# patrickltobing/shallow-wavenet

Hardware: AMD Instinct MI355X
Metric: decoded samples/sec (22.05 kHz Laplacian AR decode, whole job) (higher is better)
Workload: dtype f32

## Files before the change

shallow_wavenet_amd/csrc/swn_decode_bl6w.hip:

```cpp
#include <type_traits>
#include "swn_decode_bl6_common.hpp"
#include "swn_decode_internal.hpp"

#ifndef SWN_RES_SLICE
#define SWN_RES_SLICE 0
#endif
#ifndef SWN_ROTATE
#define SWN_ROTATE 1
#endif

namespace {

using namespace swn_bl6;

constexpr int NG = 256;
constexpr int S = 128;
constexpr int O1 = 128;

template <int LPC_, bool EXT_>
struct Tw {
    static constexpr int LPC = LPC_;
    static constexpr bool EXT = EXT_;
    using Ext = Tw<LPC_, true>;
    static constexpr int NO = 2 + LPC_;
    static constexpr int WN = cmax(1, LPC_) + 1;
    static constexpr int ring_len(int l) { return pow2ceil((1 << l) + 1); }
    static constexpr int ring_off(int l) { int o = 0; for (int i = 0; i < l; ++i) o += ring_len(i) * H; return o; }
    static constexpr int PF = L * 2 * H;
    static constexpr int NZC = 64, NZB = 4;
    static constexpr int o_ring = 0;
    static constexpr int o_hcat = o_ring + ring_off(L);
    static constexpr int o_gp = o_hcat + L * H;
    static constexpr int o_bx = o_gp + 2 * PF;
    static constexpr int o_bd = o_bx + L * 2 * H;
    static constexpr int o_old = o_bd + L * 2 * H;
    static constexpr int o_wup = o_old + 2 * L * 2 * H;
    static constexpr int o_skip = o_wup + 256;
    static constexpr int o_p2 = o_skip + S;
    static constexpr int o_tnz = o_p2 + 4 * NO;
    static constexpr int o_cz = o_tnz + r4(NZB * NZC);
    static constexpr int o_w2 = o_cz + 5 * H;
    static constexpr int o_bias = o_w2 + NO * S + r4(NO);
    static constexpr int o_w1 = o_bias + S + O1;
    static constexpr int o_wl = o_w1 + 8 * O1 * 16;
    static constexpr int o_h0w = o_wl + 8 * NG * 4;
    static constexpr int o_end = o_h0w + 3 * H;
    static constexpr size_t lds_bytes = (size_t)o_end * sizeof(float);
    static constexpr int sess_old = ring_off(L);
    static constexpr int sess_win = sess_old + 2 * L * 2 * H;
    static constexpr int sess_floats = sess_win + r4(WN);
};

__device__ __forceinline__ float sum_quads(float v) {
    v += dpp_f<0x124>(v);
    v += dpp_f<0x128>(v);
    float w = v;
    asm("s_nop 1\n\tv_permlane16_swap_b32 %0, %1" : "+v"(v), "+v"(w));
    v += w;
    w = v;
    asm("s_nop 1\n\tv_permlane32_swap_b32 %0, %1" : "+v"(v), "+v"(w));
    return v + w;
}
__device__ __forceinline__ float quad_sum_by_parity(float own, float other) {
    float s = own + dpp_f<0xB1>(other);
    s += dpp_f<0x4E>(s);
    return s;
}
struct NoWork { __device__ __forceinline__ void operator()() const {} };
template <class T, int LAYER, int NQ = 2, class BEHIND = NoWork>
__device__ __forceinline__ void layer_a(float* lds, const float (&w)[2][16], const int q, const float wj, const int pb, const int po,
                                        const int ta, const float* xr, BEHIND&& behind = NoWork{}) {
    constexpr bool ROT = !std::is_same<typename std::decay<BEHIND>::type, NoWork>::value;
    const int o = ta >> 2, p = ta & 3, pr = p & 1;
    const float e_old = lds[T::o_old + po + LAYER * 2 * H + pr * H + o];
    const float g_gp = lds[T::o_gp + pb + LAYER * 2 * H + pr * H + o], g_bx = lds[T::o_bx + LAYER * 2 * H + pr * H + o];
    const float e_hp = xr[o];
    static_assert(NQ >= 0 && NQ <= 4, "early quads");
    float4 xq[4];
    if constexpr (ROT) {
#pragma unroll
        for (int m = 0; m < NQ; ++m) xq[m] = *reinterpret_cast<const float4*>(xr + 16 * p + 4 * m);
        __builtin_amdgcn_sched_barrier(0);
        behind();
        __builtin_amdgcn_sched_barrier(0);
    }
    const float e_gx = fmaf(wj, g_gp, g_bx);
    float az = 0.f, ac = 0.f;
#pragma unroll
    for (int m = 0; m < 4; ++m) {
        float4 x;
        if (ROT && m < NQ) x = xq[m];
        else x = *reinterpret_cast<const float4*>(xr + 16 * p + 4 * m);
        az = fmaf(w[0][4 * m], x.x, az); ac = fmaf(w[1][4 * m], x.x, ac);
        az = fmaf(w[0][4 * m + 1], x.y, az); ac = fmaf(w[1][4 * m + 1], x.y, ac);
        az = fmaf(w[0][4 * m + 2], x.z, az); ac = fmaf(w[1][4 * m + 2], x.z, ac);
        az = fmaf(w[0][4 * m + 3], x.w, az); ac = fmaf(w[1][4 * m + 3], x.w, ac);
    }
    const float sq = quad_sum_by_parity(pr ? ac : az, pr ? az : ac);
    __builtin_amdgcn_sched_barrier(0);
    if (p < 2) {
        const float sa = sq + e_old;
        const float v = e_gx * sa;
        const float e = exp_c(p == 0 ? -v : -2.f * fminf(fabsf(v), 64.f));
        const float r = rcp_c(1.f + e);
        const float res = p == 0 ? r : copysignf((1.f - e) * r, v);
        const float c = dpp_f<0xF5>(res);
        if (p == 0) {
            const float hn = (1.f - res) * c + res * e_hp;
            if (LAYER + 1 < L) {
                constexpr int R2 = T::ring_len(LAYER + 1 < L ? LAYER + 1 : LAYER);
                lds[T::o_ring + T::ring_off(LAYER + 1 < L ? LAYER + 1 : LAYER) + (q & (R2 - 1)) * H + o] = hn;
            }
            lds[T::o_hcat + LAYER * H + o] = hn;
        }
    }
    __builtin_amdgcn_sched_barrier(0);
}

template <class T, int LAYER, int MB = 4>
__device__ __forceinline__ void older_sum(const float* lds, const float (&w)[2][16], const int qn, const int tb, float& az, float& ac) {
    constexpr int dil = 1 << LAYER;
    constexpr int R = T::ring_len(LAYER);
    const int p = tb & 3;
    const float* ring = lds + T::o_ring + T::ring_off(LAYER);
    az = 0.f; ac = 0.f;
#pragma unroll
    for (int m = 0; m < 4; ++m) {
        const float4 x = *reinterpret_cast<const float4*>(ring + ((qn - dil) & (R - 1)) * H + 16 * p + 4 * m);
        float4 w0, w1;
        if (LAYER < L - 1) {
            w0 = make_float4(w[0][4 * m], w[0][4 * m + 1], w[0][4 * m + 2], w[0][4 * m + 3]);
            w1 = make_float4(w[1][4 * m], w[1][4 * m + 1], w[1][4 * m + 2], w[1][4 * m + 3]);
        } else {
            w0 = *reinterpret_cast<const float4*>(lds + T::o_wl + (m * NG + tb) * 4);
            w1 = *reinterpret_cast<const float4*>(lds + T::o_wl + ((4 + m) * NG + tb) * 4);
        }
        az = fmaf(w0.x, x.x, az); ac = fmaf(w1.x, x.x, ac);
        az = fmaf(w0.y, x.y, az); ac = fmaf(w1.y, x.y, ac);
        az = fmaf(w0.z, x.z, az); ac = fmaf(w1.z, x.z, ac);
        az = fmaf(w0.w, x.w, az); ac = fmaf(w1.w, x.w, ac);
        if (MB < 4 && m % MB == MB - 1) __builtin_amdgcn_sched_barrier(0);
    }
    az = sum4(az); ac = sum4(ac);
}
template <class T, int LAYER>
__device__ __forceinline__ void older_store(float* lds, const int qn, const int tb, const float az, const float ac) {
    const int o = tb >> 2, p = tb & 3, pr = p & 1;
    lds[T::o_old + (qn & 1) * (L * 2 * H) + LAYER * 2 * H + pr * H + o] = (p == 0 ? az : ac) + lds[T::o_bd + LAYER * 2 * H + pr * H + o];
}
template <class T, int LAYER, int MB = 4>
__device__ __forceinline__ void older_b(float* lds, const float (&w)[2][16], const int qn, const int tb) {
    float az, ac;
    older_sum<T, LAYER, MB>(lds, w, qn, tb, az, ac);
    if ((tb & 3) < 2) older_store<T, LAYER>(lds, qn, tb, az, ac);
}
template <class T>
__device__ __forceinline__ void older_last_rows(const float* lds, const int qn, const int tb, float4 (&x)[2], float4 (&w)[2][2]) {
    constexpr int LAYER = L - 1, dil = 1 << LAYER, R = T::ring_len(LAYER);
    const float* row = lds + T::o_ring + T::ring_off(LAYER) + ((qn - dil) & (R - 1)) * H + 16 * (tb & 3);
#pragma unroll
    for (int m = 0; m < 2; ++m) {
        x[m] = *reinterpret_cast<const float4*>(row + 4 * m);
        w[m][0] = *reinterpret_cast<const float4*>(lds + T::o_wl + (m * NG + tb) * 4);
        w[m][1] = *reinterpret_cast<const float4*>(lds + T::o_wl + ((4 + m) * NG + tb) * 4);
    }
}
template <class T>
__device__ __forceinline__ void older_last_x(float* lds, const float4 (&xe)[2], const float4 (&we)[2][2], const int qn, const int tb) {
    constexpr int LAYER = L - 1, dil = 1 << LAYER, R = T::ring_len(LAYER);
    const float* row = lds + T::o_ring + T::ring_off(LAYER) + ((qn - dil) & (R - 1)) * H + 16 * (tb & 3);
    float az = 0.f, ac = 0.f;
#pragma unroll
    for (int m = 0; m < 4; ++m) {
        float4 x, w0, w1;
        if (m < 2) { x = xe[m]; w0 = we[m][0]; w1 = we[m][1]; }
        else {
            x = *reinterpret_cast<const float4*>(row + 4 * m);
            w0 = *reinterpret_cast<const float4*>(lds + T::o_wl + (m * NG + tb) * 4);
            w1 = *reinterpret_cast<const float4*>(lds + T::o_wl + ((4 + m) * NG + tb) * 4);
        }
        az = fmaf(w0.x, x.x, az); ac = fmaf(w1.x, x.x, ac);
        az = fmaf(w0.y, x.y, az); ac = fmaf(w1.y, x.y, ac);
        az = fmaf(w0.z, x.z, az); ac = fmaf(w1.z, x.z, ac);
        az = fmaf(w0.w, x.w, az); ac = fmaf(w1.w, x.w, ac);
        if (m == 1) __builtin_amdgcn_sched_barrier(0);
    }
    az = sum4(az); ac = sum4(ac);
    if ((tb & 3) < 2) older_store<T, LAYER>(lds, qn, tb, az, ac);
}
template <int... LS> struct Layers {};
template <class T, int NW, int... LS>
__device__ __forceinline__ void older_bn(Layers<LS...>, float* lds, const float (&w)[NW][2][16], const int qn, const int tb) {
    static_assert(((LS < NW) && ...), "register-resident halves only");
    float az[sizeof...(LS)], ac[sizeof...(LS)];
    int k = 0;
    ((older_sum<T, LS>(lds, w[LS], qn, tb, az[k], ac[k]), ++k), ...);
    if ((tb & 3) < 2) {
        k = 0;
        ((older_store<T, LS>(lds, qn, tb, az[k], ac[k]), ++k), ...);
    }
}

template <class T, int LAYER>
__device__ __forceinline__ void older_rows(const float* lds, const int qn, const int tb, float4 (&x)[4]) {
    constexpr int dil = 1 << LAYER;
    constexpr int R = T::ring_len(LAYER);
    const float* row = lds + T::o_ring + T::ring_off(LAYER) + ((qn - dil) & (R - 1)) * H + 16 * (tb & 3);
#pragma unroll
    for (int m = 0; m < 4; ++m) x[m] = *reinterpret_cast<const float4*>(row + 4 * m);
}
__device__ __forceinline__ void older_sum_x(const float (&w)[2][16], const float4 (&x)[4], float& az, float& ac) {
    az = 0.f; ac = 0.f;
#pragma unroll
    for (int m = 0; m < 4; ++m) {
        az = fmaf(w[0][4 * m], x[m].x, az); ac = fmaf(w[1][4 * m], x[m].x, ac);
        az = fmaf(w[0][4 * m + 1], x[m].y, az); ac = fmaf(w[1][4 * m + 1], x[m].y, ac);
        az = fmaf(w[0][4 * m + 2], x[m].z, az); ac = fmaf(w[1][4 * m + 2], x[m].z, ac);
        az = fmaf(w[0][4 * m + 3], x[m].w, az); ac = fmaf(w[1][4 * m + 3], x[m].w, ac);
    }
    az = sum4(az); ac = sum4(ac);
}
template <class T, int... LS>
__device__ __forceinline__ void older_rows_n(Layers<LS...>, const float* lds, const int qn, const int tb, float4 (&x)[sizeof...(LS)][4]) {
    int k = 0;
    ((older_rows<T, LS>(lds, qn, tb, x[k]), ++k), ...);
}
template <class T, int NW, int... LS>
__device__ __forceinline__ void older_bn_x(Layers<LS...>, float* lds, const float (&w)[NW][2][16], const float4 (&x)[sizeof...(LS)][4],
                                           const int qn, const int tb) {
    static_assert(((LS < NW) && ...), "register-resident halves only");
    float az[sizeof...(LS)], ac[sizeof...(LS)];
    int k = 0;
    ((older_sum_x(w[LS], x[k], az[k], ac[k]), ++k), ...);
    if ((tb & 3) < 2) {
        k = 0;
        ((older_store<T, LS>(lds, qn, tb, az[k], ac[k]), ++k), ...);
    }
}

template <int LAYER>
__device__ __forceinline__ void skip_issue_b(__amdgpu_buffer_rsrc_t wsk2, float4 (&wsl)[8], const int tb, const unsigned step0) {
    const int r = tb >> 2, hp = tb & 3;
#pragma unroll
    for (int ps = 0; ps < 2; ++ps)
#pragma unroll
        for (int mm = 0; mm < 4; ++mm)
            wsl[ps * 4 + mm] = buf_ld4(wsk2, (unsigned)((r + 64 * ps) * 4 + hp) * 16u, (unsigned)((LAYER * 4 + mm) * S) * 64u + step0);
}
template <class T, int LAYER, bool REQ = true>
__device__ __forceinline__ void skip_roll_b(const float* lds, __amdgpu_buffer_rsrc_t wsk2, const float4 (&wcur)[8], float4 (&wnext)[8],
                                            float (&sacc)[2], const int tb, const unsigned step0) {
    static_assert(LAYER >= 1 && LAYER < L, "slice LAYER - 1 in flight, slice LAYER to request");
    const int r = tb >> 2, hp = tb & 3;
    float4 xs[4];
#pragma unroll
    for (int mm = 0; mm < 4; ++mm) xs[mm] = *reinterpret_cast<const float4*>(lds + T::o_hcat + (LAYER - 1) * H + 16 * mm + 4 * hp);
#pragma unroll
    for (int mm = 0; mm < 4; ++mm) {
#pragma unroll
        for (int ps = 0; ps < 2; ++ps) {
            const float4 x = xs[mm], w = wcur[ps * 4 + mm];
            sacc[ps] = fmaf(w.x, x.x, sacc[ps]); sacc[ps] = fmaf(w.y, x.y, sacc[ps]);
            sacc[ps] = fmaf(w.z, x.z, sacc[ps]); sacc[ps] = fmaf(w.w, x.w, sacc[ps]);
        }
        __builtin_amdgcn_sched_barrier(0);
#pragma unroll
        for (int ps = 0; ps < 2; ++ps)
            if (REQ) wnext[ps * 4 + mm] = buf_ld4(wsk2, (unsigned)((r + 64 * ps) * 4 + hp) * 16u, (unsigned)((LAYER * 4 + mm) * S) * 64u + step0);
        __builtin_amdgcn_sched_barrier(0);
    }
    asm volatile("" : "+v"(sacc[0]), "+v"(sacc[1]));
}
template <class T>
__device__ __forceinline__ void skip_last_b(float* lds, const float4 (&wsl)[8], const float (&sacc)[2], const int tb) {
    const int r = tb >> 2, hp = tb & 3;
    float part[2][4];
#pragma unroll
    for (int mm = 0; mm < 4; ++mm) {
        const float4 x = *reinterpret_cast<const float4*>(lds + T::o_hcat + (L - 1) * H + 16 * mm + 4 * hp);
#pragma unroll
        for (int ps = 0; ps < 2; ++ps) {
            const float4 w = wsl[ps * 4 + mm];
            part[ps][mm] = fmaf(w.w, x.w, fmaf(w.z, x.z, fmaf(w.y, x.y, w.x * x.x)));
        }
    }
    float s[2];
#pragma unroll
    for (int ps = 0; ps < 2; ++ps) s[ps] = sacc[ps] + ((part[ps][0] + part[ps][1]) + (part[ps][2] + part[ps][3]));
    const float t0 = s[0] + dpp_f<0xB1>(s[0]), t1 = s[1] + dpp_f<0xB1>(s[1]);
    const float v = (hp < 2 ? t0 : t1) + dpp_f<0x4E>(hp < 2 ? t1 : t0);
    if ((hp & 1) == 0) lds[T::o_skip + r + 32 * hp] = fmaxf(v, 0.f);
}

using OlderMerged = Layers<3, 4>;
using OlderOut1 = Layers<0, 1, 2>;

template <class T, bool GA, bool STREAM, bool POOL = false>
__device__ __forceinline__ void decode_body(const Bl6Args& a, float* lds) {
    constexpr bool EXT = T::EXT;
    static_assert(!STREAM || EXT, "streamed chunks run the extended mode");
    constexpr bool grpA = GA;
    const int tid = threadIdx.x, b = POOL ? 0 : blockIdx.x;
    __builtin_assume(GA ? tid < NG : tid >= NG);
    const int tg = tid & (NG - 1);
    const float* __restrict__ P = a.P;
    const int U = a.U;
    const int s0 = STREAM ? a.step0 : 0;
    const bool resume = STREAM && a.resume;
    const int fb0 = STREAM ? s0 / U : 0;

    for (int e = tid; e < T::o_end; e += NT) lds[e] = 0.f;
    __syncthreads();
    for (int e = tid; e < L * 2 * H; e += NT) {
        lds[T::o_bx + e] = P[a.y.bx + e];
        const float bd = P[a.y.bd + e];
        lds[T::o_bd + e] = bd;
        lds[T::o_old + e] = bd;
    }
    for (int e = tid; e < U; e += NT) lds[T::o_wup + e] = P[a.y.wup + e];
    for (int e = tid; e < H; e += NT) lds[T::o_cz + e] = P[a.y.cb + e];
    for (int e = tid; e < S; e += NT) lds[T::o_bias + e] = P[a.y.bsk + e];
    for (int e = tid; e < O1; e += NT) lds[T::o_bias + S + e] = P[a.y.b1 + e];
    for (int e = tid; e < 2 * H; e += NT) { lds[T::o_cz + H + e] = P[a.y.cv + e]; lds[T::o_cz + 3 * H + e] = P[a.y.cc + e]; }
    for (int e = tid; e < T::NO * S; e += NT) lds[T::o_w2 + e] = P[a.y.w2 + (size_t)(e / S) * r4(S) + (e % S)];
    for (int e = tid; e < T::NO; e += NT) lds[T::o_w2 + T::NO * S + e] = P[a.y.b2 + e];
    for (int e = tid; e < 8 * O1 * 16; e += NT) lds[T::o_w1 + e] = P[a.y.w12 + e];
    const __amdgpu_buffer_rsrc_t condr =
        make_rsrc(a.cond + (size_t)b * a.Tf * a.N, (unsigned)((size_t)a.Tf * a.N * sizeof(float)));
    auto load_frame = [&](int fr) {
        float* dst = lds + T::o_gp + (fr & 1) * T::PF;
#pragma unroll
        for (int it = 0; it < (T::PF / 4 + NT - 1) / NT; ++it) {
            const int e4 = it * NT + tid;
            if (e4 < T::PF / 4)
                *reinterpret_cast<float4*>(dst + 4 * e4) =
                    buf_ld4(condr, (unsigned)tid * 16u, (unsigned)(fr * a.N * 4 + it * NT * 16));
        }
    };
    for (int fr = fb0; fr < fb0 + 2 && fr < a.Tf; ++fr) load_frame(fr);
    constexpr int NWR = grpA ? L : L - 1;
    float wreg[NWR][2][16];
    {
        const int o = tg >> 2, p = tg & 3, k = grpA ? 1 : 0;
#pragma unroll
        for (int l = 0; l < L; ++l)
#pragma unroll
            for (int r = 0; r < 2; ++r) {
                const float4* src = reinterpret_cast<const float4*>(P + a.y.wd + (((size_t)l * 2 * H + o + r * H) * 2 + k) * H + 16 * p);
#pragma unroll
                for (int v = 0; v < 4; ++v) {
                    const float4 t = src[v];
                    if (l == L - 1 && !grpA) {
                        *reinterpret_cast<float4*>(lds + T::o_wl + ((r * 4 + v) * NG + tg) * 4) = t;
                    } else {
                        float (&wr)[16] = wreg[l < NWR ? l : 0][r];
                        wr[4 * v] = t.x; wr[4 * v + 1] = t.y; wr[4 * v + 2] = t.z; wr[4 * v + 3] = t.w;
                    }
                }
            }
    }
    __syncthreads();
    const float* sess_b = STREAM ? a.sess + (size_t)b * T::sess_floats : nullptr;
    int tcp = tid;
    asm volatile("" : "+v"(tcp));
    if (resume) {
        for (int e = tcp; e < T::ring_off(L); e += NT) lds[T::o_ring + e] = sess_b[e];
        for (int e = tcp; e < 2 * L * 2 * H; e += NT) lds[T::o_old + e] = sess_b[T::sess_old + e];
        __syncthreads();
    }

    int fb = fb0, tb0 = fb0 * U;
    const int n_pro = RF;
    auto cond_taps = [&](int q, float& wj, int& pb) {
        const int t0 = q - RF;
        const int tlo = t0 < 0 ? 0 : t0;
        if (tlo >= tb0 + U) {
            fb += 1; tb0 += U;
            if (fb + 1 < a.Tf) load_frame(fb + 1);
        }
        int rel = tlo - tb0;
        int fsel = fb;
        if (rel >= U) { rel -= U; fsel = fb + 1; }
        rel = rel < U ? rel : U - 1;
        wj = lds[T::o_wup + rel];
        pb = (fsel & 1) * T::PF;
    };

    auto input_seed = [&](int q) {
        if (tid < H) {
            const int o = tid;
            float acc = c_b;
#pragma unroll
            for (int k = 0; k < 2; ++k) {
                const int r = q - (1 - k);
                if (r >= 0) acc += fmaf(k ? c_v1 : c_v0, 0.f, k ? c_c1 : c_c0);
            }
            lds[T::o_ring + (q & 1) * H + o] = ssign(acc);
        }
    };
    float win[T::WN];
#pragma unroll
    for (int k = 0; k < T::WN; ++k) win[k] = 0.f;
    if (EXT && a.seed) win[T::WN - 1] = reinterpret_cast<const float*>(a.seed)[b];
    if (resume) {
#pragma unroll
        for (int k = 0; k < T::WN; ++k) win[k] = sess_b[T::sess_win + k];
    }
    const int wv = __builtin_amdgcn_readfirstlane(tg >> 6);
    float kcb = 0.f, kv0 = 0.f, kv1 = 0.f, kc0 = 0.f, kc1 = 0.f;
    if (grpA) { const int o = tg & (H - 1); kcb = c_b; kv0 = c_v0; kv1 = c_v1; kc0 = c_c0; kc1 = c_c1; }
    auto h0_row = [&](int qn) -> int {
        return wv == 0 ? T::o_ring + (qn & 1) * H : T::o_h0w + (wv - 1) * H;
    };
    auto input_gen = [&](int row) {
        if constexpr (grpA) {
            float acc = kcb;
            acc += fmaf(kv0, win[T::WN - 2], kc0);
            acc += fmaf(kv1, win[T::WN - 1], kc1);
            lds[row + (tg & (H - 1))] = ssign(acc);
            lds_fence_compiler();
        }
    };
    float e_next = 0.f;
    auto noise_load = [&](int c) {
        const int step = c * T::NZC + tid - 64;
        if (step < a.n_steps) e_next = a.noise[(size_t)b * a.n_steps + step];
    };
    auto noise_chunk = [&](int c) {
        if (grpA && tid >= 64 && tid < 128) {
            const int k = tid - 64, step = c * T::NZC + k;
            if (step < a.n_steps) {
                const float e = EXT ? swn_noise_laplace_at(a.nz, b, step, s0 + step, 0, a.n_steps, 1) : e_next;
                const float sg = (e > 0.f) ? 1.f : ((e < 0.f) ? -1.f : 0.f);
                lds[T::o_tnz + (c & (T::NZB - 1)) * T::NZC + k] = sg * log1pf(-2.f * fabsf(e));
            }
            if (!EXT) noise_load(c + 1);
        }
    };
    if (!EXT && grpA && tid >= 64 && tid < 128) noise_load(0);
    noise_chunk(0);
    noise_chunk(1);

    const __amdgpu_buffer_rsrc_t wsk2 = make_rsrc(P + a.y.wsk2, (unsigned)(L * S * 64 * sizeof(float)));
    constexpr bool NEWFORM = !EXT && T::LPC == 0;
    constexpr int RES = (grpA || !NEWFORM) ? -1 : SWN_RES_SLICE;
    static_assert(RES == -1 || RES == 0 || RES == L - 1, "the first or the last slice");
    float4 wres[8];
    if constexpr (RES == 0) skip_issue_b<0>(wsk2, wres, tg, 0u);
    if constexpr (RES == L - 1) skip_issue_b<L - 1>(wsk2, wres, tg, 0u);

#ifdef SWN_STAMP
    unsigned long long tw[9] = {0, 0, 0, 0, 0, 0, 0, 0, 0}, tv[6] = {0, 0, 0, 0, 0, 0}, tstep = 0, tlast = 0, tbeg = 0;
#define SWN_BAR(k) { tw[k] += __builtin_amdgcn_s_memtime() - tlast; lds_barrier(); tlast = __builtin_amdgcn_s_memtime(); }
#define SWN_WAIT_STAMP(k) { asm volatile("" :: "v"(wsl[0].x)); tv[k] += __builtin_amdgcn_s_memtime() - tlast; }
#define SWN_PRE(k) { tw[k] += __builtin_amdgcn_s_memtime() - tlast; asm volatile("s_waitcnt lgkmcnt(0)" ::: "memory"); }
#define SWN_BAR_KEEP(k, N) { lds_barrier_keep<N>(); tlast = __builtin_amdgcn_s_memtime(); }
#else
#define SWN_BAR(k) lds_barrier();
#define SWN_WAIT_STAMP(k)
#define SWN_PRE(k)
#define SWN_BAR_KEEP(k, N) lds_barrier_keep<N>();
#endif
#define SWN_PHASE_WORK(LAYER, GEN, X0)                                                                                \
    if constexpr (grpA) layer_a<T, LAYER>(lds, wreg[LAYER], q, wj, pb, po, tg,                                         \
                                          LAYER == 0 ? (X0) : lds + T::o_ring + T::ring_off(LAYER) +                   \
                                                                  (q & (T::ring_len(LAYER) - 1)) * H);                 \
    else {                                                                                                             \
        if (GEN) {    \
                      \
                      \
                      \
            if (LAYER == 0) { if (RES != 0) skip_issue_b<0>(wsk2, wsl, tg, step0); }                                   \
            else if (LAYER == 1 && RES == 0) skip_roll_b<T, 1>(lds, wsk2, wres, wsl, sacc, tg, step0);                 \
            else { SWN_WAIT_STAMP(LAYER > 0 ? LAYER - 1 : 0)                                                           \
                   skip_roll_b<T, (LAYER > 0 ? LAYER : 1), !(LAYER == L - 1 && RES == L - 1)>(lds, wsk2, wsl, wsl, sacc, tg, step0); } \
            __builtin_amdgcn_sched_barrier(0);                                                                         \
        }                                                                                                              \
        if (!(GEN)) older_b<T, LAYER>(lds, wreg[LAYER < NWR ? LAYER : 0], q + 1, tg);                                  \
        else if (LAYER == 0) older_bn<T>(OlderMerged{}, lds, wreg, q + 1, tg);                                         \
        __builtin_amdgcn_sched_barrier(0);                                                                             \
    }
#define SWN_PHASE(LAYER, GEN, X0) SWN_PHASE_WORK(LAYER, GEN, X0) if (GEN) { SWN_BAR(LAYER) } else lds_barrier();

#pragma unroll 1
    for (int q = resume ? n_pro : 0; q < n_pro; ++q) {
        float wj; int pb;
        float4 wsl[8]; float sacc[2]; const unsigned step0 = 0;
        cond_taps(q, wj, pb);
        const int po = (q & 1) * (L * 2 * H);
        input_seed(q);
        lds_barrier();
        const float* x0 = lds + T::o_ring + (q & 1) * H;
        SWN_PHASE(0, false, x0) SWN_PHASE(1, false, x0) SWN_PHASE(2, false, x0) SWN_PHASE(3, false, x0)
        SWN_PHASE(4, false, x0) SWN_PHASE(5, false, x0)
        (void)wsl; (void)sacc; (void)step0;
    }

    int rel_c = s0 - fb0 * U;
    bool fill_c = false;
    float wj_c = 0.f;
    int pb_c = 0, po_c = 0, x0_c = 0;
    auto taps_ahead = [&](int qn) {
        wj_c = lds[T::o_wup + rel_c];
        pb_c = (fb & 1) * T::PF;
        po_c = (qn & 1) * (L * 2 * H);
        x0_c = h0_row(qn);
        asm volatile("" : "+s"(pb_c), "+s"(po_c), "+s"(x0_c));
    };
    auto frame_advance = [&]() {
        rel_c += 1;
        const bool cross = rel_c >= U;
        if (cross) { rel_c = 0; fb += 1; }
        fill_c = cross && fb + 1 < a.Tf;
    };
    if constexpr (grpA) taps_ahead(RF + s0);
    input_gen(x0_c);
#ifdef SWN_STAMP
    tlast = tbeg = __builtin_amdgcn_s_memtime();
#endif
    constexpr bool ROT = SWN_ROTATE && NEWFORM;
    constexpr int ROTQ = 2;
    float sv_p = 0.f, acc_p = 0.f;
    const __amdgpu_buffer_rsrc_t outr =
        make_rsrc(reinterpret_cast<float*>(a.out) + (size_t)b * a.n_steps, (unsigned)((size_t)a.n_steps * sizeof(float)));
    const __amdgpu_buffer_rsrc_t headr =
        make_rsrc(HEADS_ON && a.heads ? a.heads + (size_t)b * a.n_steps * T::NO : nullptr,
                  HEADS_ON && a.heads ? (unsigned)((size_t)a.n_steps * T::NO * sizeof(float)) : 0u);
    auto store_step = [&](const int ip) __attribute__((always_inline)) {
        if constexpr (grpA && ROT) {
            if (tid == 0) __builtin_amdgcn_raw_buffer_store_b32(__builtin_bit_cast(unsigned, sv_p), outr, 0u, (unsigned)ip * 4u, 0);
            if (wv == 0 && (tg & 63) < T::NO)
                __builtin_amdgcn_raw_buffer_store_b32(__builtin_bit_cast(unsigned, acc_p), headr, (unsigned)(tg & 63) * 4u,
                                                      (unsigned)(ip * T::NO) * 4u, 0);
        } else if constexpr (grpA) {
            if (tid == 0) reinterpret_cast<float*>(a.out)[(size_t)b * a.n_steps + (size_t)ip] = sv_p;
            if (HEADS_ON && a.heads && wv == 0 && (tg & 63) < T::NO) a.heads[((size_t)b * a.n_steps + ip) * T::NO + (tg & 63)] = acc_p;
        }
    };
    auto gen_step = [&](const int i) __attribute__((always_inline)) {
        const int q = RF + s0 + i;
        const float wj = wj_c;
        const int pb = pb_c, po = po_c;
        if constexpr (grpA && !ROT) {
            if (fill_c) load_frame(fb + 1);
        }
        auto behind0 = [&]() __attribute__((always_inline)) {
            if ((i & (T::NZC - 1)) == 0) noise_chunk((i >> 6) + 2);
            if (fill_c) load_frame(fb + 1);
            if (i > 0) store_step(i - 1);
        };
        float4 wsl[8];
        float sacc[2] = {0.f, 0.f};
        if constexpr (!grpA) {
            const float bs0 = lds[T::o_bias + (tg >> 2)], bs1 = lds[T::o_bias + (tg >> 2) + 64];
            if ((tg & 3) == 0) { sacc[0] = bs0; sacc[1] = bs1; }
        }
        unsigned step0 = 0;
        asm volatile("" : "+s"(step0));
        const float* x0 = lds + x0_c;
        if constexpr (grpA && ROT) {
            layer_a<T, 0, ROTQ>(lds, wreg[0], q, wj, pb, po, tg, x0, behind0);
            SWN_BAR(0)
        } else {
            SWN_PHASE(0, true, x0)
        }
        SWN_PHASE(1, true, x0) SWN_PHASE(2, true, x0) SWN_PHASE(3, true, x0)
        SWN_PHASE(4, true, x0)
        constexpr bool EARLY5 = T::LPC == 0;
        float4 xl[2], wl[2][2];
        SWN_PHASE_WORK(5, true, x0)
        if constexpr (grpA && EARLY5) {
            SWN_PRE(5)
            lds_fence_compiler();
            __builtin_amdgcn_sched_barrier(0);
            older_last_rows<T>(lds, q + 1, tg + (int)step0, xl, wl);
            __builtin_amdgcn_sched_barrier(0);
            SWN_BAR_KEEP(5, 6)
        } else {
            SWN_BAR(5)
        }
        constexpr bool ROLL1 = T::LPC == 0;
        float4 xo[3][4];
        float4 w1e[2][2];
        if constexpr (!grpA) {
            if constexpr (RES == L - 1) skip_last_b<T>(lds, wres, sacc, tg);
            else { SWN_WAIT_STAMP(5) skip_last_b<T>(lds, wsl, sacc, tg); }
            SWN_PRE(6)
            lds_fence_compiler();
            __builtin_amdgcn_sched_barrier(0);
            older_rows_n<T>(OlderOut1{}, lds, q + 1, tg, xo);
            __builtin_amdgcn_sched_barrier(0);
            SWN_BAR_KEEP(6, 12)
        } else {
            if constexpr (EARLY5) older_last_x<T>(lds, xl, wl, q + 1, tg + (int)step0);
            else older_b<T, L - 1, 2>(lds, wreg[L - 1], q + 1, tg + (int)step0);
            if constexpr (ROLL1) {
                SWN_PRE(6)
                lds_fence_compiler();
                __builtin_amdgcn_sched_barrier(0);
#pragma unroll
                for (int mm = 0; mm < 2; ++mm)
#pragma unroll
                    for (int r = 0; r < 2; ++r)
                        w1e[mm][r] = *reinterpret_cast<const float4*>(lds + T::o_w1 + ((mm * O1 + (tg >> 2) + 64 * r) * 4 + (tg & 3)) * 4);
                __builtin_amdgcn_sched_barrier(0);
                SWN_BAR_KEEP(6, 4)
            } else {
                SWN_BAR(6)
            }
        }
        if constexpr (grpA) {
            const int hr = tg >> 2, hp = tg & 3;
            float a0 = 0.f, a1 = 0.f, b0 = 0.f, b1 = 0.f;
            auto X = [&](int mm) { return *reinterpret_cast<const float4*>(lds + T::o_skip + 16 * mm + 4 * hp); };
            auto W = [&](int mm, int r) { return *reinterpret_cast<const float4*>(lds + T::o_w1 + ((mm * O1 + hr + 64 * r) * 4 + hp) * 4); };
            auto fma8 = [&](int mm, const float4& x0, const float4& w0, const float4& w1) {
                float& acc = (mm & 1) ? a1 : a0;
                float& bcc = (mm & 1) ? b1 : b0;
                acc = fmaf(w0.x, x0.x, acc); acc = fmaf(w0.y, x0.y, acc); acc = fmaf(w0.z, x0.z, acc); acc = fmaf(w0.w, x0.w, acc);
                bcc = fmaf(w1.x, x0.x, bcc); bcc = fmaf(w1.y, x0.y, bcc); bcc = fmaf(w1.z, x0.z, bcc); bcc = fmaf(w1.w, x0.w, bcc);
            };
            float e_b1[2] = {0.f, 0.f}, e_w2[2] = {0.f, 0.f}, e_b2 = 0.f;
            const int e_kc = hp < T::NO ? hp : T::NO - 1;
            if constexpr (ROLL1) {
                static_assert(T::NO <= 4, "one round of out_2 rows");
                float4 xr[3] = {X(0), X(1), X(2)};
                __builtin_amdgcn_sched_barrier(0);
#pragma unroll
                for (int mm = 0; mm < 8; ++mm) {
                    fma8(mm, xr[mm % 3], w1e[mm % 2][0], w1e[mm % 2][1]);
                    __builtin_amdgcn_sched_barrier(0);
                    if (mm + 2 < 8) { w1e[mm % 2][0] = W(mm + 2, 0); w1e[mm % 2][1] = W(mm + 2, 1); }
                    if (mm + 3 < 8) xr[mm % 3] = X(mm + 3);
                    if (mm == 5) {
                        e_b1[0] = lds[T::o_bias + S + hr]; e_b1[1] = lds[T::o_bias + S + hr + 64];
                        e_w2[0] = lds[T::o_w2 + e_kc * S + hr]; e_w2[1] = lds[T::o_w2 + e_kc * S + hr + 64];
                    }
                    if (mm == 6) e_b2 = lds[T::o_w2 + T::NO * S + e_kc];
                    __builtin_amdgcn_sched_barrier(0);
                }
            } else {
#pragma unroll
                for (int mm = 0; mm < 8; ++mm) {
                    fma8(mm, X(mm), W(mm, 0), W(mm, 1));
                    if ((mm & 3) == 3) __builtin_amdgcn_sched_barrier(0);
                }
            }
            const float v = sum4(a0 + a1), u = sum4(b0 + b1);
            if constexpr (ROLL1) {
                const float o1a = fmaxf(v + e_b1[0], 0.f), o1b = fmaxf(u + e_b1[1], 0.f);
                const float pz = sum_quads(fmaf(e_w2[1], o1b, fmaf(e_w2[0], o1a, tg < 4 ? e_b2 : 0.f)));
                if ((tg & 63) < 4 && hp < T::NO) lds[T::o_p2 + 4 * hp + wv] = pz;
            } else {
                const float o1a = fmaxf(v + lds[T::o_bias + S + hr], 0.f), o1b = fmaxf(u + lds[T::o_bias + S + hr + 64], 0.f);
#pragma unroll
                for (int j = 0; j < (T::NO + 3) / 4; ++j) {
                    const int k = hp + 4 * j, kc = k < T::NO ? k : T::NO - 1;
                    const float* w2 = lds + T::o_w2 + kc * S;
                    const float b2 = lds[T::o_w2 + T::NO * S + kc];
                    const float pz = sum_quads(fmaf(w2[hr + 64], o1b, fmaf(w2[hr], o1a, tg < 4 ? b2 : 0.f)));
                    if ((tg & 63) < 4 && k < T::NO) lds[T::o_p2 + 4 * k + wv] = pz;
                }
            }
        } else {
            older_bn_x<T>(OlderOut1{}, lds, wreg, xo, q + 1, tg);
        }
        SWN_BAR(7)
        if constexpr (grpA) {
            const int ln = tg & 63;
            float tz = 0.f;
            if constexpr (!EXT) tz = lds[T::o_tnz + (i & (T::NZB * T::NZC - 1))];
            float fv = 0.f;
            if (a.forced) fv = reinterpret_cast<const float*>(a.forced)[(size_t)b * a.n_steps + i];
            const float4 pz = *reinterpret_cast<const float4*>(lds + T::o_p2 + 4 * (ln < T::NO ? ln : T::NO - 1));
            __builtin_amdgcn_sched_barrier(0);
            frame_advance();
            taps_ahead(q + 1);
            __builtin_amdgcn_sched_barrier(0);
            const float acc = (pz.x + pz.y) + (pz.z + pz.w);
            float o2[T::NO];
#pragma unroll
            for (int k = 0; k < T::NO; ++k) o2[k] = __builtin_bit_cast(float, __builtin_amdgcn_readlane(__builtin_bit_cast(int, acc), k));
            float sv;
            {
#pragma clang fp contract(off)
                const float mu = o2[0];
                const float bsc = sigm(o2[1]);
                float lpv = 0.f;
#pragma unroll
                for (int k = 0; k < T::LPC; ++k) lpv += o2[2 + T::LPC - 1 - k] * win[T::WN - T::LPC + k];
                const float t = bsc * (EXT ? lds[T::o_tnz + ((i >> 6) & (T::NZB - 1)) * T::NZC + (i & (T::NZC - 1))] : tz);
                sv = (T::LPC > 0) ? (lpv + mu) - t : mu - t;
                sv = fminf(fmaxf(sv, -1.f), 1.f);
                float fd = a.forced ? fv : sv;
                asm volatile("" : "+v"(fd));
#pragma unroll
                for (int k = 0; k + 1 < T::WN; ++k) win[k] = win[k + 1];
                win[T::WN - 1] = fd;
            }
            if (i + 1 < a.n_steps) input_gen(x0_c);
            __builtin_amdgcn_sched_barrier(0);
            if constexpr (ROT) { sv_p = sv; acc_p = acc; }
            else {
                if (tid == 0) reinterpret_cast<float*>(a.out)[(size_t)b * a.n_steps + (size_t)i] = sv;
                if (HEADS_ON && a.heads && wv == 0 && ln < T::NO) a.heads[((size_t)b * a.n_steps + i) * T::NO + ln] = acc;
            }
        }
#ifdef SWN_STAMP
        if constexpr (grpA) tw[8] += __builtin_amdgcn_s_memtime() - tlast;
#endif
    };
    if constexpr (ROT) {
#pragma unroll 1
        for (int i = 0; i < a.n_steps; ++i) gen_step(i);
        if (a.n_steps > 0) store_step(a.n_steps - 1);
    } else {
#pragma unroll 1
        for (int i0 = 0; i0 < a.n_steps; i0 += T::NZC) {
            noise_chunk((i0 >> 6) + 2);
            const int iend = i0 + T::NZC < a.n_steps ? i0 + T::NZC : a.n_steps;
#pragma unroll 1
            for (int i = i0; i < iend; ++i) gen_step(i);
        }
    }
#ifdef SWN_STAMP
    { const unsigned long long tn = __builtin_amdgcn_s_memtime(); tw[0] += tn - tlast; tstep = tn - tbeg; }
#endif
    if constexpr (STREAM) {
        __syncthreads();
        float* so = a.sess + (size_t)b * T::sess_floats;
        tcp = tid;
        asm volatile("" : "+v"(tcp));
        for (int e = tcp; e < T::ring_off(L); e += NT) so[e] = lds[T::o_ring + e];
        for (int e = tcp; e < 2 * L * 2 * H; e += NT) so[T::sess_old + e] = lds[T::o_old + e];
        if (tid == 0) {
#pragma unroll
            for (int k = 0; k < T::WN; ++k) so[T::sess_win + k] = win[k];
        }
    }
#undef SWN_PHASE
#undef SWN_PHASE_WORK
#undef SWN_BAR
#undef SWN_WAIT_STAMP
#undef SWN_PRE
#undef SWN_BAR_KEEP
#ifdef SWN_STAMP
    if ((tid == 0 || tid == 64 || tid == NG) && b == 0 && a.heads) {
        float* h = a.heads + (tid == 0 ? 0 : tid == 64 ? 30 : 10);
        for (int k = 0; k < 9; ++k) h[k] = (float)((double)tw[k] / (double)a.n_steps);
        if (tid == 0) h[9] = (float)((double)tstep / (double)a.n_steps);
        else if (tid == NG) for (int k = 0; k < 6; ++k) h[10 + k] = (float)((double)tv[k] / (double)a.n_steps);
    }
#endif
}

template <class T, bool STREAM = false>
__global__ __launch_bounds__(NT) void decode_bl6w_kernel(const Bl6Args a) {
    extern __shared__ __attribute__((aligned(16))) float lds[];
    if (threadIdx.x < NG) decode_body<T, true, STREAM>(a, lds);
    else decode_body<T, false, STREAM>(a, lds);
}

template <class T, bool MODELS = false>
__global__ __launch_bounds__(NT) void decode_bl6w_pool_kernel(
    const typename std::conditional<MODELS, Bl6PoolModelsArgs, Bl6PoolArgs>::type p) {
    extern __shared__ __attribute__((aligned(16))) float lds[];
    static_assert(T::EXT, "pools run the extended mode");
    Bl6Args a = p.c;
    if constexpr (MODELS) a.P = swn_pool_model(p.m);
    if (!swn_pool_entry_args(a, p.t, 1, 1, T::NO)) return;
    a.sess += (size_t)swn_pool_slot(p.t) * T::sess_floats;
    if (threadIdx.x < NG) decode_body<T, true, true, true>(a, lds);
    else decode_body<T, false, true, true>(a, lds);
}

bool bl6w_applies(const SwnGeom& g) {
    return g.bl6 && g.U <= 256 && g.U >= 2 && !g.audio_in && g.kind == SWN_KIND_LAPLACE && g.S == 128 && g.O1 == 128 &&
           g.seg == 1 && (g.lpc == 0 || g.lpc == 4);
}

template <class F>
int with_tw(const SwnGeom& g, F&& f) {
    if (!bl6w_applies(g)) return SWN_E_UNSUPPORTED;
    if (g.lpc == 0) return f(Tw<0, false>{});
    return f(Tw<4, false>{});
}

}

int swn_decode_bl6w_run(const SwnDecodeCall& c) {
    const hipStream_t st = c.hip_stream;
    if (c.pool) {
        Bl6PoolModelsArgs p;
        fill_args(p.c, c);
        p.t = *c.pool;
        if (c.models) p.m = *c.models;
        return with_tw(c.g, [&](auto tw) {
            using T = typename decltype(tw)::Ext;
            if (c.models)
                return launch_kernel(decode_bl6w_pool_kernel<T, true>, T::lds_bytes, c.batch, p, st, "swn_decode_pool_chunk_models(bl6w)");
            const Bl6PoolArgs& p1 = p;
            return launch_kernel(decode_bl6w_pool_kernel<T>, T::lds_bytes, c.batch, p1, st, "swn_decode_pool_chunk(bl6w)");
        });
    }
    Bl6Args a;
    fill_args(a, c);
    return with_tw(c.g, [&](auto t) {
        using T = decltype(t);
        using X = typename T::Ext;
        static_assert(T::lds_bytes <= 160 * 1024 && X::lds_bytes <= 160 * 1024, "LDS budget");
        if (c.stream) return launch_kernel(decode_bl6w_kernel<X, true>, X::lds_bytes, a.B, a, st, "swn_decode(bl6w)");
        if (wants_ext(a)) return launch_kernel(decode_bl6w_kernel<X>, X::lds_bytes, a.B, a, st, "swn_decode(bl6w)");
        return launch_kernel(decode_bl6w_kernel<T>, T::lds_bytes, a.B, a, st, "swn_decode(bl6w)");
    });
}

size_t swn_decode_bl6w_session_floats(const SwnGeom& g) {
    int n = 0;
    with_tw(g, [&](auto t) { n = decltype(t)::sess_floats; return SWN_OK; });
    return (size_t)n;
}
```

Baseline: 403,600.

## Move older layer 2 into merged group-B pass and add optional side-work handoff

Measured after the change: 408,800 (median of 6 runs). 1.3% higher.

```diff
diff --git a/shallow_wavenet_amd/csrc/swn_decode_bl6w.hip b/shallow_wavenet_amd/csrc/swn_decode_bl6w.hip
--- a/shallow_wavenet_amd/csrc/swn_decode_bl6w.hip
+++ b/shallow_wavenet_amd/csrc/swn_decode_bl6w.hip
@@ -7,6 +7,15 @@
 #endif
 #ifndef SWN_ROTATE
 #define SWN_ROTATE 1
+#endif
+#ifndef SWN_HANDOFF
+#define SWN_HANDOFF 0
+#endif
+#ifndef SWN_OLDER2_MERGED
+#define SWN_OLDER2_MERGED 1
+#endif
+#ifndef SWN_EARLY_ROWS
+#define SWN_EARLY_ROWS 1
 #endif
 
 namespace {
@@ -22,6 +31,7 @@
     static constexpr int LPC = LPC_;
     static constexpr bool EXT = EXT_;
     using Ext = Tw<LPC_, true>;
+    static constexpr bool NEWFORM = !EXT_ && LPC_ == 0;
     static constexpr int NO = 2 + LPC_;
     static constexpr int WN = cmax(1, LPC_) + 1;
     static constexpr int ring_len(int l) { return pow2ceil((1 << l) + 1); }
@@ -44,7 +54,9 @@
     static constexpr int o_w1 = o_bias + S + O1;
     static constexpr int o_wl = o_w1 + 8 * O1 * 16;
     static constexpr int o_h0w = o_wl + 8 * NG * 4;
-    static constexpr int o_end = o_h0w + 3 * H;
+    static constexpr int o_ho = o_h0w + 3 * H;
+    static constexpr int HO = 4, NHO = 128;
+    static constexpr int o_end = o_ho + (NEWFORM && (SWN_HANDOFF & 1) && SWN_ROTATE ? NHO * HO : 0);
     static constexpr size_t lds_bytes = (size_t)o_end * sizeof(float);
     static constexpr int sess_old = ring_off(L);
     static constexpr int sess_win = sess_old + 2 * L * 2 * H;
@@ -292,8 +304,12 @@
     if ((hp & 1) == 0) lds[T::o_skip + r + 32 * hp] = fmaxf(v, 0.f);
 }
 
-using OlderMerged = Layers<3, 4>;
-using OlderOut1 = Layers<0, 1, 2>;
+template <bool MOVE2> using OlderMergedT = typename std::conditional<MOVE2, Layers<2, 3, 4>, Layers<3, 4>>::type;
+template <bool MOVE2> using OlderOut1T = typename std::conditional<MOVE2, Layers<0, 1>, Layers<0, 1, 2>>::type;
+template <int E> struct Out1Split;
+template <> struct Out1Split<2> { using Early = Layers<0, 1>; using Late = Layers<>; };
+template <> struct Out1Split<1> { using Early = Layers<0>; using Late = Layers<1>; };
+template <> struct Out1Split<0> { using Early = Layers<>; using Late = Layers<0, 1>; };
 
 template <class T, bool GA, bool STREAM, bool POOL = false>
 __device__ __forceinline__ void decode_body(const Bl6Args& a, float* lds) {
@@ -421,14 +437,34 @@
             lds_fence_compiler();
         }
     };
+#ifdef SWN_DIAG_NOSIDE
+    constexpr bool NOSIDE = T::NEWFORM;
+#else
+    constexpr bool NOSIDE = false;
+#endif
+#ifdef SWN_DIAG_NOSTREAM
+    constexpr bool NOSTREAM = T::NEWFORM;
+#else
+    constexpr bool NOSTREAM = false;
+#endif
+    constexpr bool HOFF = T::NEWFORM && (SWN_HANDOFF & 7) && SWN_ROTATE;
+    constexpr bool HO_ST = HOFF && (SWN_HANDOFF & 1), HO_RF = HOFF && (SWN_HANDOFF & 2), HO_NZ = HOFF && (SWN_HANDOFF & 4);
+    constexpr bool MOVE2 = T::NEWFORM && SWN_OLDER2_MERGED;
+    using OlderMerged = OlderMergedT<MOVE2>;
+    using OlderOut1 = OlderOut1T<MOVE2>;
+    constexpr int NOUT1 = MOVE2 ? 2 : 3;
+    constexpr int NEARLY = MOVE2 ? SWN_EARLY_ROWS : NOUT1;
+    static_assert(NEARLY >= 0 && NEARLY <= NOUT1, "early rows");
+    constexpr bool NZG = HO_NZ ? !grpA : grpA;
+    const int tn = HO_NZ ? tg : tid;
     float e_next = 0.f;
     auto noise_load = [&](int c) {
-        const int step = c * T::NZC + tid - 64;
+        const int step = c * T::NZC + tn - 64;
         if (step < a.n_steps) e_next = a.noise[(size_t)b * a.n_steps + step];
     };
     auto noise_chunk = [&](int c) {
-        if (grpA && tid >= 64 && tid < 128) {
-            const int k = tid - 64, step = c * T::NZC + k;
+        if (NZG && tn >= 64 && tn < 128) {
+            const int k = tn - 64, step = c * T::NZC + k;
             if (step < a.n_steps) {
                 const float e = EXT ? swn_noise_laplace_at(a.nz, b, step, s0 + step, 0, a.n_steps, 1) : e_next;
                 const float sg = (e > 0.f) ? 1.f : ((e < 0.f) ? -1.f : 0.f);
@@ -437,12 +473,12 @@
             if (!EXT) noise_load(c + 1);
         }
     };
-    if (!EXT && grpA && tid >= 64 && tid < 128) noise_load(0);
+    if (!EXT && NZG && tn >= 64 && tn < 128) noise_load(0);
     noise_chunk(0);
     noise_chunk(1);
 
     const __amdgpu_buffer_rsrc_t wsk2 = make_rsrc(P + a.y.wsk2, (unsigned)(L * S * 64 * sizeof(float)));
-    constexpr bool NEWFORM = !EXT && T::LPC == 0;
+    constexpr bool NEWFORM = T::NEWFORM;
     constexpr int RES = (grpA || !NEWFORM) ? -1 : SWN_RES_SLICE;
     static_assert(RES == -1 || RES == 0 || RES == L - 1, "the first or the last slice");
     float4 wres[8];
@@ -471,9 +507,9 @@
                       \
                       \
             if (LAYER == 0) { if (RES != 0) skip_issue_b<0>(wsk2, wsl, tg, step0); }                                   \
-            else if (LAYER == 1 && RES == 0) skip_roll_b<T, 1>(lds, wsk2, wres, wsl, sacc, tg, step0);                 \
+            else if (LAYER == 1 && RES == 0) skip_roll_b<T, 1, !NOSTREAM>(lds, wsk2, wres, wsl, sacc, tg, step0);      \
             else { SWN_WAIT_STAMP(LAYER > 0 ? LAYER - 1 : 0)                                                           \
-                   skip_roll_b<T, (LAYER > 0 ? LAYER : 1), !(LAYER == L - 1 && RES == L - 1)>(lds, wsk2, wsl, wsl, sacc, tg, step0); } \
+                   skip_roll_b<T, (LAYER > 0 ? LAYER : 1), !(LAYER == L - 1 && RES == L - 1) && !NOSTREAM>(lds, wsk2, wsl, wsl, sacc, tg, step0); } \
             __builtin_amdgcn_sched_barrier(0);                                                                         \
         }                                                                                                              \
         if (!(GEN)) older_b<T, LAYER>(lds, wreg[LAYER < NWR ? LAYER : 0], q + 1, tg);                                  \
@@ -537,6 +573,31 @@
             if (HEADS_ON && a.heads && wv == 0 && (tg & 63) < T::NO) a.heads[((size_t)b * a.n_steps + ip) * T::NO + (tg & 63)] = acc_p;
         }
     };
+    static_assert(!HOFF || (T::PF / 4 <= NG && T::NO == 2 && T::HO == 4), "one refill request per thread, a slot is {head, head, sample, -}");
+    auto ho_write = [&](const int ip) __attribute__((always_inline)) {
+        if constexpr (grpA) {
+            if (wv == 0) {
+                float* const slot = lds + T::o_ho + (ip & (T::NHO - 1)) * T::HO;
+                slot[(tg & 63) < T::NO ? (tg & 63) : T::NO - 1] = acc_p;
+                slot[T::NO] = sv_p;
+            }
+        }
+    };
+    auto load_frame_b = [&](int fr) {
+        if (tg < T::PF / 4)
+            *reinterpret_cast<float4*>(lds + T::o_gp + (fr & 1) * T::PF + 4 * tg) =
+                buf_ld4(condr, (unsigned)tg * 16u, (unsigned)(fr * a.N * 4));
+    };
+    auto store_chunk_b = [&](const int c) __attribute__((always_inline)) {
+        const int step = c * 64 + tg;
+        if (tg < 64 && step < a.n_steps) {
+            const float4 v = *reinterpret_cast<const float4*>(lds + T::o_ho + (step & (T::NHO - 1)) * T::HO);
+            __builtin_amdgcn_raw_buffer_store_b32(__builtin_bit_cast(unsigned, v.z), outr, (unsigned)tg * 4u, (unsigned)c * 256u, 0);
+            using u2 = unsigned __attribute__((ext_vector_type(2)));
+            u2 h; h.x = __builtin_bit_cast(unsigned, v.x); h.y = __builtin_bit_cast(unsigned, v.y);
+            __builtin_amdgcn_raw_buffer_store_b64(h, headr, (unsigned)tg * 8u, (unsigned)c * 512u, 0);
+        }
+    };
     auto gen_step = [&](const int i) __attribute__((always_inline)) {
         const int q = RF + s0 + i;
         const float wj = wj_c;
@@ -545,9 +606,11 @@
             if (fill_c) load_frame(fb + 1);
         }
         auto behind0 = [&]() __attribute__((always_inline)) {
-            if ((i & (T::NZC - 1)) == 0) noise_chunk((i >> 6) + 2);
-            if (fill_c) load_frame(fb + 1);
-            if (i > 0) store_step(i - 1);
+            if constexpr (NOSIDE) return;
+            if constexpr (!HO_NZ) { if ((i & (T::NZC - 1)) == 0) noise_chunk((i >> 6) + 2); }
+            if constexpr (!HO_RF) { if (fill_c) load_frame(fb + 1); }
+            if constexpr (HO_ST) { if (i > 0) ho_write(i - 1); }
+            else { if (i > 0) store_step(i - 1); }
         };
         float4 wsl[8];
         float sacc[2] = {0.f, 0.f};
@@ -558,6 +621,22 @@
         unsigned step0 = 0;
         asm volatile("" : "+s"(step0));
         const float* x0 = lds + x0_c;
+#ifdef SWN_DIAG_NOSIDE_B
+        constexpr bool SIDE_B = false;
+#else
+        constexpr bool SIDE_B = HOFF && !grpA && !NOSIDE;
+#endif
+        if constexpr (SIDE_B) {
+            __builtin_amdgcn_sched_barrier(0);
+            if constexpr (HO_NZ) { if ((i & (T::NZC - 1)) == 0) noise_chunk((i >> 6) + 2); }
+            if constexpr (HO_RF) { if (fill_c) load_frame_b(fb + 1); }
+            if constexpr (HO_ST) { if ((i & 63) == 1 && i > 1) store_chunk_b((i >> 6) - 1); }
+            __builtin_amdgcn_sched_barrier(0);
+        }
+        if constexpr (NOSTREAM && !grpA) {
+#pragma unroll
+            for (int k = 0; k < 8; ++k) asm volatile("" : "=v"(wsl[k].x), "=v"(wsl[k].y), "=v"(wsl[k].z), "=v"(wsl[k].w));
+        }
         if constexpr (grpA && ROT) {
             layer_a<T, 0, ROTQ>(lds, wreg[0], q, wj, pb, po, tg, x0, behind0);
             SWN_BAR(0)
@@ -580,7 +659,8 @@
             SWN_BAR(5)
         }
         constexpr bool ROLL1 = T::LPC == 0;
-        float4 xo[3][4];
+        using Split = Out1Split<MOVE2 ? NEARLY : 2>;
+        float4 xo[cmax(NEARLY, 1)][4];
         float4 w1e[2][2];
         if constexpr (!grpA) {
             if constexpr (RES == L - 1) skip_last_b<T>(lds, wres, sacc, tg);
@@ -588,9 +668,17 @@
             SWN_PRE(6)
             lds_fence_compiler();
             __builtin_amdgcn_sched_barrier(0);
-            older_rows_n<T>(OlderOut1{}, lds, q + 1, tg, xo);
-            __builtin_amdgcn_sched_barrier(0);
-            SWN_BAR_KEEP(6, 12)
+            if constexpr (!MOVE2) {
+                older_rows_n<T>(OlderOut1{}, lds, q + 1, tg, xo);
+                __builtin_amdgcn_sched_barrier(0);
+                SWN_BAR_KEEP(6, 12)
+            } else if constexpr (NEARLY > 0) {
+                older_rows_n<T>(typename Split::Early{}, lds, q + 1, tg, xo);
+                __builtin_amdgcn_sched_barrier(0);
+                SWN_BAR_KEEP(6, 4 * NEARLY)
+            } else {
+                SWN_BAR_KEEP(6, 0)
+            }
         } else {
             if constexpr (EARLY5) older_last_x<T>(lds, xl, wl, q + 1, tg + (int)step0);
             else older_b<T, L - 1, 2>(lds, wreg[L - 1], q + 1, tg + (int)step0);
@@ -662,8 +750,11 @@
                     if ((tg & 63) < 4 && k < T::NO) lds[T::o_p2 + 4 * k + wv] = pz;
                 }
             }
+        } else if constexpr (!MOVE2) {
+            older_bn_x<T>(OlderOut1{}, lds, wreg, xo, q + 1, tg);
         } else {
-            older_bn_x<T>(OlderOut1{}, lds, wreg, xo, q + 1, tg);
+            if constexpr (NEARLY > 0) older_bn_x<T>(typename Split::Early{}, lds, wreg, xo, q + 1, tg);
+            if constexpr (NEARLY < NOUT1) older_bn<T>(typename Split::Late{}, lds, wreg, q + 1, tg);
         }
         SWN_BAR(7)
         if constexpr (grpA) {
@@ -706,6 +797,7 @@
                 if (HEADS_ON && a.heads && wv == 0 && ln < T::NO) a.heads[((size_t)b * a.n_steps + i) * T::NO + ln] = acc;
             }
         }
+        if constexpr (HO_RF && !grpA) frame_advance();
 #ifdef SWN_STAMP
         if constexpr (grpA) tw[8] += __builtin_amdgcn_s_memtime() - tlast;
 #endif
@@ -713,7 +805,13 @@
     if constexpr (ROT) {
 #pragma unroll 1
         for (int i = 0; i < a.n_steps; ++i) gen_step(i);
-        if (a.n_steps > 0) store_step(a.n_steps - 1);
+        if constexpr (HO_ST) {
+            if constexpr (grpA) { if (a.n_steps > 0) ho_write(a.n_steps - 1); }
+            lds_barrier();
+            if constexpr (!grpA) {
+                for (int c = a.n_steps >= 66 ? ((a.n_steps - 66) >> 6) + 1 : 0; c * 64 < a.n_steps; ++c) store_chunk_b(c);
+            }
+        } else if (a.n_steps > 0) store_step(a.n_steps - 1);
     } else {
 #pragma unroll 1
         for (int i0 = 0; i0 < a.n_steps; i0 += T::NZC) {
```
